# qxiaofan/awesome-orb-slam3-3dvisioncraft-version

Measured on AMD Instinct MI355X. Metric: frames/sec ORB extract+match (752×480, 1000 kp) + LocalBA iters/sec; 1/2/4/8 GPU, higher is better.
Workload: dtype u8

## Files before the change

### awesome-orb-slam3-3dvisioncraft-version_amd/_abi.py

```python
import ctypes as C

import numpy as np

ORB_OK, ORB_E_EMPTY_IMAGE, ORB_E_CAPACITY, ORB_E_INVALID, ORB_E_HIP, ORB_E_NOMEM, ORB_E_ABORTED = 0, -1, -2, -3, -4, -5, -6

KP_DTYPE = np.dtype([("x", "<f4"), ("y", "<f4"), ("size", "<f4"), ("angle", "<f4"), ("response", "<f4"),
                     ("octave", "<i4"), ("class_id", "<i4")])


class OrbxConfig(C.Structure):
    _fields_ = [("nfeatures", C.c_int32), ("scale_factor", C.c_float), ("nlevels", C.c_int32),
                ("ini_th_fast", C.c_int32), ("min_th_fast", C.c_int32)]


TH_HIGH, TH_LOW, HISTO_LENGTH = 100, 50, 30
GRID_COLS, GRID_ROWS = 64, 48
MODE_LOCAL_MAP, MODE_BEST_ONLY, MODE_INIT = 0, 1, 2
Q_VALID, Q_STEREO, Q_HAS_OBS, Q_RIGHT, Q_TWIN = 1, 2, 4, 8, 16

QUERY_DTYPE = np.dtype([("u", "<f4"), ("v", "<f4"), ("radius", "<f4"), ("u_right", "<f4"), ("angle", "<f4"),
                        ("min_level", "<i2"), ("max_level", "<i2"), ("flags", "<u4")])


class GridParams(C.Structure):
# ... 439 lines not shown
    "ORBM_LBA_R_NUM_FIXED_KF": LBA_R_NUM_FIXED_KF, "ORBM_LBA_R_N_POINTS": LBA_R_N_POINTS, "ORBM_LBA_R_N_EDGES": LBA_R_N_EDGES,
    "ORBM_LBA_R_N_MONO": LBA_R_N_MONO, "ORBM_LBA_R_N_STEREO": LBA_R_N_STEREO, "ORBM_LBA_R_N_POSES_REQUIRED": LBA_R_N_POSES_REQUIRED,
    "ORBM_LBA_R_N_POINTS_REQUIRED": LBA_R_N_POINTS_REQUIRED, "ORBM_LBA_R_N_EDGES_REQUIRED": LBA_R_N_EDGES_REQUIRED,
    "ORBM_LBA_R_WORDS": LBA_R_WORDS, "ORBM_LBA_BAD_INDEX": LBA_BAD_INDEX, "ORBM_LBA_UNSUPPORTED": LBA_UNSUPPORTED,
    "ORBM_LBA_OVERFLOW": LBA_OVERFLOW, "ORBM_LBA_EARLY_RETURN": LBA_EARLY_RETURN, "ORBM_LBA_A_FLAGS": LBA_A_FLAGS,
    "ORBM_LBA_A_N_ERASED": LBA_A_N_ERASED, "ORBM_LBA_A_N_WENT_BAD": LBA_A_N_WENT_BAD, "ORBM_LBA_A_N_OBS": LBA_A_N_OBS,
    "ORBM_LBA_A_N_MONO": LBA_A_N_MONO, "ORBM_LBA_A_N_STEREO": LBA_A_N_STEREO, "ORBM_LBA_A_WORDS": LBA_A_WORDS,
    "BOWDB_KF_PRESENT": KF_PRESENT, "BOWDB_COVIS": COVIS, "BOWDB_MAX_CANDIDATES": MAX_CANDIDATES, "BOWDB_L1_NORM": BOWDB_L1_NORM,
    "LBA_EDGE_MONO": EDGE_MONO, "LBA_EDGE_STEREO": EDGE_STEREO, "LBA_EDGE_BODY": EDGE_BODY, "LBA_CAM_PINHOLE": CAM_PINHOLE, "LBA_CAM_KB8": CAM_KB8,
    "LBA_HINT_MONO_PINHOLE": HINT_MONO_PINHOLE, "LBA_HINT_PINHOLE": HINT_PINHOLE, "LIBA_MAX_FREE": LIBA_MAX_FREE, "LIBA_EDGE_CLOSE": EDGE_CLOSE,
}


def _prototypes():
    vp, i32, u32, sz, f32, f64, P = C.c_void_p, C.c_int, C.c_uint, C.c_size_t, C.c_float, C.c_double, C.POINTER
    lba, liba = P(LbaProblem), P(LibaProblem)
    return {
        "orbx_create": (i32, [P(OrbxConfig), i32, i32, i32, i32, P(vp)]),
        "orbx_destroy": (None, [vp]),
        "orbx_last_error": (C.c_char_p, [vp]),
        "orbx_get_tables": (i32, [vp, vp, vp, vp, vp, vp]),
        "orbx_max_keypoints": (i32, [vp]),
        "orbx_extract": (i32, [vp, vp, i32, i32, i32, i32, i32, vp, vp, i32, P(i32), P(i32)]),
        "orbx_extract_view": (i32, [vp, vp, i32, i32, i32, i32, i32, P(vp), P(vp), P(i32), P(i32)]),
        "orbx_set_host_pyramid": (i32, [vp, i32]),
        "orbx_host_pyramid_level": (i32, [vp, i32, P(vp), P(i32), P(i32), P(i32)]),
        "orbx_extract_batch_dev": (i32, [vp, vp, i32, sz, i32, i32, i32, vp, vp, i32, vp, vp]),
        "orbx_pyramid_level": (i32, [vp, i32, i32, P(vp), P(i32), P(i32), P(i32)]),
        "orbx_copy_level": (i32, [vp, i32, i32, i32, vp]),
        "orbx_stereo_matches": (i32, [vp, vp, vp, vp, vp, vp, vp, vp, i32, i32, f32, f32, vp, vp, vp, vp]),
        "orbx_stereo_matches_last": (i32, [vp, vp, f32, f32, vp, vp, i32, P(i32)]),
        "orbx_debug_candidates": (i32, [vp, i32, i32, vp, i32, P(i32)]),
        "orbx_debug_selected": (i32, [vp, i32, i32, vp, i32, P(i32)]),
        "orbx_enable_timing": (i32, [vp, i32]),
        "orbx_last_timing": (i32, [vp, vp]),
        "orbx_last_fast_passes": (i32, [vp, vp, vp, vp]),
        "orbx_last_schedule": (i32, [vp, P(i32), P(i32)]),

        "orbm_hamming": (i32, [vp, i32, vp, i32, i32, vp, vp]),
        "orbm_knn2": (i32, [vp, vp, i32, vp, vp, i32, i32, i32, vp, vp, vp]),
        "orbm_grid_build": (i32, [vp, vp, i32, i32, i32, P(GridParams), vp, vp, vp]),
        "orbm_search_workspace_bytes": (sz, [i32, i32]),
        "orbm_search_by_projection": (i32, [vp, vp, vp, vp, vp, i32, i32, vp, vp, vp, vp, vp, i32, i32, P(SearchParams), vp, vp, vp, vp, vp]),
        "orbm_search_by_bow": (i32, [P(BowSide), vp, P(BowSide), i32, f32, i32, vp, vp, vp]),
        "orbm_search_by_bow_kf": (i32, [P(BowSide), vp, P(BowSide), vp, i32, f32, i32, vp, vp, vp]),
        "orbm_enable_timing": (i32, [i32]),
        "orbm_last_timing": (i32, [vp]),
        "orbm_grid_build_rig": (i32, [vp, vp, vp, i32, i32, i32, P(GridParams), vp, vp, vp]),
        "orbm_search_by_projection_rig": (i32, [vp, vp, vp, vp, vp, i32, i32, vp, vp, vp, vp, vp, i32, i32, P(SearchParams), vp, vp, vp, vp, vp]),
        "orbm_fuse": (i32, [vp, vp, vp, vp, i32, i32, vp, vp, vp, vp, vp, i32, i32, P(FuseParams), vp, vp, vp, vp]),
        "orbm_search_for_triangulation": (i32, [P(TriSide), P(TriSide), vp, i32, i32, i32, i32, vp, vp, vp]),
        "orbm_search_for_triangulation_kb8": (i32, [P(TriSide), P(TriSide), vp, vp, vp, i32, i32, i32, i32, vp, vp, vp]),
        "orbm_mutual_matches": (i32, [vp, vp, vp, vp, i32, i32, i32, vp, vp, vp]),
        "orbm_predict_scale_thresholds": (i32, [f32, i32, vp]),
        "orbm_project_map_points": (i32, [vp, vp, i32, vp, vp, i32, P(ProjectParams), vp, vp, vp, vp, vp, vp, vp, i32, vp]),
        "orbm_refresh_map_points": (i32, [vp, i32, vp, i32, vp, i32, vp, vp, vp, vp, i32, vp, i32, P(RefreshParams), vp, vp, vp]),
        "orbm_create_new_map_points": (i32, [P(NewPtSide), P(NewPtSide), vp, vp, i32, vp, vp, i32, vp, vp, vp, vp, vp, vp]),
        "orbm_append_new_map_points": (i32, [vp, vp, i32, vp, i32, vp, i32, vp, vp, i32, i32, vp, vp, i32, vp, vp, i32, vp, vp]),
        "orbm_local_map_workspace_bytes": (sz, [i32, i32, i32]),
        "orbm_update_local_map": (i32, [P(LocalMapView), vp, P(LocalMapLists), i32, P(LocalMapOut), vp, vp]),
        "orbm_store_local_tracks": (i32, [vp, vp, vp, i32, i32, vp, i32, i32, vp]),
        "orbm_cull_workspace_bytes": (sz, [i32, i32, i32, i32]),
        "orbm_cull_workspace": (i32, [i32, i32, i32, P(CullWorkspaceLayout)]),
        "orbm_cull_keyframes": (i32, [P(LocalMapView), P(CullIn), i32, P(CullOut), vp, vp]),
        "orbm_apply_keyframe_culling": (i32, [P(LocalMapView), P(CullIn), i32, i32, P(CullApply), vp, vp]),
        "orbm_covis_workspace_bytes": (sz, [i32, i32]),
# ... 73 lines not shown
```

### awesome-orb-slam3-3dvisioncraft-version_amd/csrc/orbx_extractor.hip

```cpp
#include <hip/hip_runtime.h>

#include <climits>

#include <cfloat>
#include <cmath>
#include <cstdint>
#include <cstdio>
#include <cstring>
#include <string>
#include <type_traits>
#include <vector>

#include "../../include/orbhip.h"
#include "lds_optin.inc"
#include <mutex>

#define ORBX_MAX_LEVELS 16
#ifdef ORBX_PROF
__device__ unsigned long long g_prof[2][8][256];
#define PROF_DECL unsigned long long prof_t = clock64(), prof_d[8] = {0, 0, 0, 0, 0, 0, 0, 0}
#define PROF_MARK(k, slot) do { const unsigned long long t_ = clock64(); prof_d[slot] += t_ - prof_t; prof_t = t_; } while (0)
#define PROF_FLUSH(k) do { if ((threadIdx.x & 63) < 8) atomicAdd(&g_prof[k][threadIdx.x & 7][(blockIdx.x * 4 + (threadIdx.x >> 6)) & 255], prof_d[threadIdx.x & 7]); } while (0)
#else
#define PROF_DECL do {} while (0)
#define PROF_MARK(k, slot) do {} while (0)
#define PROF_FLUSH(k) do {} while (0)
#endif
#define ORBX_EVENTS_ON(h) ((h)->timing && !(h)->capturing)
#define ORBX_EDGE 19
#define ORBX_MINB 16
#define FAST_QCAP 2048
#define FAST_MAXCELLS 32

static const int8_t h_pattern[1024] = {
#include "orb_pattern.inc"
};
static __constant__ float4 c_patternf[256];
static __constant__ int c_umax[16];
static __constant__ uint32_t c_div16[16] = {0, 65536, 32768, 21846, 16384, 13108, 10923, 9363, 8192, 7282, 6554, 5958, 5462, 5042, 4682, 4370};
static __constant__ uint32_t c_icmask[16][12];

static __device__ __forceinline__ bool xcd_frame_unit_m(const int unitsPerFrame, const uint32_t magic, const int batch, int* frame, int* unit, const int lead = 0, const bool reverse = false) {
    const int xcd = blockIdx.x & 7;
    const uint32_t slot = (uint32_t)(blockIdx.x - lead) >> 3;
    const uint32_t q0 = magic ? (uint32_t)(((unsigned long long)slot * magic) >> 32) : slot / (uint32_t)unitsPerFrame;
    const uint32_t q = reverse ? (uint32_t)((batch + 7) >> 3) - 1u - q0 : q0;
    const int fr = (int)q * 8 + xcd;
    *frame = fr;
    *unit = (int)(slot - q0 * (uint32_t)unitsPerFrame);
    return fr < batch;
}
static inline uint32_t xcd_units_magic(int unitsPerFrame, int batch) {
    const unsigned long long u = (unsigned long long)std::max(unitsPerFrame, 1), slots = u * (unsigned long long)((batch + 7) / 8);
    if (u < 2 || slots * u >= 0x100000000ull) return 0u;
    return (uint32_t)(0x100000000ull / u + 1ull);
}

#include "resize_window.inc"

struct ResizeParams {
    const uint8_t* src; size_t sFrame; int sStride, sw, sh;
    uint8_t* dst; size_t dFrame; int dStride, dw, dh;
    double scale_x, scale_y;
    const int* coef;
    int stripsX, stripsY;
    int stripRows, batch;
    int unitsPerFrame;
    uint32_t unitsMagic;
    int reverse;
    const Resize2Strip* strips;
    const Resize2Row* rows;
    int* ordCand; int* ordOut; uint32_t* ordHostMax; uint32_t* ordRetry; int ordLevels; uint32_t ordTiles;
// ... 646 lines not shown
        } else {
#pragma unroll
            for (int k = 0; k < NS; k++) {
                rr[k] = r; cc[k] = c;
                if (tid + 256 * k < ng) fetch(r, c, w[k]);
                r += dr; c += dc;
                if (c >= gq) { c -= gq; r++; }
            }
        }
#pragma unroll
        for (int k = 0; k < NS; k++)
            if (tid + 256 * k < ng) put(rr[k], cc[k], w[k]);
        for (int i = tid + 256 * NS; i < ng; i += 256) {
            uint32_t wx[5];
            fetch(r, c, wx);
            put(r, c, wx);
            r += dr; c += dc;
            if (c >= gq) { c -= gq; r++; }
        }
        if (tid < 8 + FAST_MAXCELLS) sh[tid] = 0;
        if (tid < detW) {
            const int cell = (int)(mul24((uint32_t)tid, (uint32_t)L.wCellMagic) >> 16);
            const int cellx0 = (int)mul24((uint32_t)cell, (uint32_t)L.wCell);
            const int cx = tid - cellx0, cw = min(L.wCell, detW - cellx0);
            colTab[tid] = (uint8_t)(cell | (cx == 0 ? 0x40 : 0) | (cx + 1 >= cw ? 0x80 : 0));
        }
    }
    PROF_MARK(0, 0);
    __syncthreads();
    PROF_MARK(0, 1);

    const int t0 = PASS == 0 ? P.iniTh : min(P.iniTh, P.minTh);
    const int wave = tid >> 6;
    const int dcol = lane & 31, rsub = lane >> 5;
    uint16_t* q1w = q1 + wave * FAST_Q1W;
    uint16_t* q2w = q2 + wave * (FAST_Q2CAP / 4);
    uint8_t* sbuf = (uint8_t*)q1w;
    static_assert(FAST_Q2CAP / 4 <= 2 * FAST_Q1W, "a wave's scores are parked in its q1 slice");
    static_assert((FAST_Q2CAP / 4 + 1) / 2 + 256 <= FAST_Q1W && FAST_FITS_MAX <= FAST_Q1W, "a row group (<= 256 survivors) queues behind the parked scores");
    static_assert(4 * FAST_PITCH <= 4 * FAST_Q1W * 2, "the fallback's four-row score ring lives in the q1 region");
    static_assert(FAST_CROWS <= 2 && FAST_MAXCELLS / FAST_CROWS <= 16, "a tile's cells are bit 16 * cell row + cell of a 32-bit mask (retry list)");
    int n2w = 0;
    bool ovf = false;
    auto classify = [&](const int i, const bool valid) {
        int ent = 0, S = 0;
        if (valid) {
            ent = q1w[i];
            S = fast_S_pk(img + (dy0 + (ent >> 8)) * pitch + dx0 + (ent & 255), pitch);
        }
        const bool corner = valid && S > t0;
        const unsigned long long mc = __ballot(corner);
        const int nc = __popcll(mc);
        if (n2w + nc <= FAST_Q2CAP / 4) {
            if (corner) {
                const int slot = n2w + __popcll(mc & ((1ull << lane) - 1ull));
                q2w[slot] = (uint16_t)ent;
                sbuf[slot] = (uint8_t)(S - 1);
            }
            n2w += nc;
        } else if (mc) ovf = true;
    };
    uint32_t KB, KG;
    fast_pretest_consts(t0, &KB, &KG);
    const int K = (detH + 7) >> 3;
    uint32_t mask = 0;
    uint32_t colMask[FAST_CROWS];
    if (PASS == 1) {
#pragma unroll
        for (int cr = 0; cr < FAST_CROWS; cr++) {
            colMask[cr] = 0;
#pragma unroll
            for (int t = 0; t < 4; t++)
                colMask[cr] |= (emitMask >> (16 * cr + (colTab[min(4 * dcol + t, detW - 1)] & 63)) & 1u) << (8 * t + 7);
        }
    }
    for (int k = 0; k < K; k++) {
        const int ry = 8 * k + 2 * wave + rsub;
        if (ry < detH && 4 * dcol < detW) {
            const uint32_t* cw = (const uint32_t*)(img + ((dy0 - 3 + ry) & 0xFF) * pitch) + dcol;
            uint32_t bits = fast_pretest4(cw, KB, KG);
            if (PASS == 1) bits &= colMask[cellRowOf(ry)];
            const int nvalid = detW - 4 * dcol;
            if (nvalid < 4) bits &= (1u << (8 * nvalid)) - 1u;
            mask |= bits >> (7 - k);
        }
    }
    {
        const int total = __builtin_amdgcn_readlane(wave_scan_incl(__popc(mask)), 63);
        const bool fits = total <= FAST_FITS_MAX;
        for (int kp = 0; kp < (fits ? 1 : K); kp++) {
            uint32_t m = fits ? mask : mask & (0x01010101u << kp);
            const int cnt = __popc(m);
            const int incl = wave_scan_incl(cnt);
            const int n1 = __builtin_amdgcn_readlane(incl, 63);
            const int qb = fits ? 0 : (n2w + 1) >> 1;
            int slot = qb + incl - cnt;
            const int ent0 = ((2 * wave + rsub) << 8) | (4 * dcol);
            while (m) {
                const int j = __ffs((int)m) - 1;
                m &= m - 1;
                q1w[slot++] = (uint16_t)(ent0 + ((j & 7) << 11) + (j >> 3));
            }
            __builtin_amdgcn_fence(__ATOMIC_RELEASE, "wavefront");
            __builtin_amdgcn_wave_barrier();
            __builtin_amdgcn_fence(__ATOMIC_ACQUIRE, "wavefront");
            for (int i0 = 0; i0 < n1; i0 += 64) classify(qb + i0 + lane, i0 + lane < n1);
            __builtin_amdgcn_fence(__ATOMIC_RELEASE, "wavefront");
            __builtin_amdgcn_wave_barrier();
            __builtin_amdgcn_fence(__ATOMIC_ACQUIRE, "wavefront");
        }
    }
    PROF_MARK(0, 2);
    if (ovf) sh[4] = 1;
    __builtin_amdgcn_fence(__ATOMIC_RELEASE, "wavefront");
    __builtin_amdgcn_wave_barrier();
    __builtin_amdgcn_fence(__ATOMIC_ACQUIRE, "wavefront");
    PROF_MARK(0, 3);
    __syncthreads();
    PROF_MARK(0, 4);
    const bool overflow = sh[4] != 0;
    int* cellCnt = sh + 8;
    auto retry_later = [&](const uint32_t cells) {
        const uint32_t i = atomicAdd(P.retry, 1u);
        P.retry[2 + 2 * i] = (uint32_t)tileIdx | ((uint32_t)frame << 16);
        P.retry[3 + 2 * i] = cells;
    };
    if (overflow && PASS == 0) { if (tid == 0) retry_later(0xFFFFFFFFu); PROF_FLUSH(0); return; }
    if (!overflow) {
        for (int i = tid; i < (P.imgBytes >> 4); i += 256) ((uint4*)smap)[i] = make_uint4(0u, 0u, 0u, 0u);
        __syncthreads();
        for (int i = lane; i < n2w; i += 64) {
            const int slot = i;
            const int ent = q2w[slot];
            const int ry = ent >> 8;
// ... 1111 lines not shown
        int run = 0, v = 0;
        for (int k = 0; k < 32; k++) { if (ctl[1] >= run && ctl[1] < run + sub[k]) v = k; run += sub[k]; }
        ctl[2] = (bin << 5) | v;
    }
    __syncthreads();
    const float median = (float)ctl[2];
    const float thDist = 1.5f * 1.4f * median;
    for (int i = tid; i < N; i += 256) {
        const int s = sad[i];
        if (s >= 0 && !((float)s < thDist)) { P.uRight[(size_t)frame * P.cap + i] = -1.0f; P.depth[(size_t)frame * P.cap + i] = -1.0f; }
    }
}

struct LevelHost {
    int w, h, stride; size_t planeOff, planeBytes;
    int maxBX, maxBY, nCols, nRows, wCell, hCell, nIni; float hX;
    int candCap; size_t candOff; int selCap, selOff;
};

struct orbx_extractor {
    orbx_config cfg; int W, H, maxBatch, device;
    std::vector<float> scale, invScale, sigma2, invSigma2; std::vector<int> nfeat; int umax[16];
    LevelHost lv[ORBX_MAX_LEVELS];
    size_t pyrFrame = 0, candFrame = 0; int selFrame = 0, nodeCap = 0, maxKp = 0;
    int nTiles = 0, nTiles1 = 0, fastImgBytes = 0, octKeyOff = 0, octMerge = 0; size_t fastSmem = 0, octSmem = 0;
    hipStream_t stream = nullptr;
    int32_t* d_rowStart = nullptr; int32_t* d_rowIdx = nullptr; int rowCapAlloc = 0;
    int4* d_chain = nullptr; int chainTiles = 0, chainBuf = 0; size_t chainSmem = 0;
    int* d_coef = nullptr; size_t coefOff[ORBX_MAX_LEVELS] = {0};
    size_t r2StripOff[ORBX_MAX_LEVELS] = {0}, r2RowOff[ORBX_MAX_LEVELS] = {0};
    uint8_t* d_pyr = nullptr; uint32_t* d_cand = nullptr; int* d_candCount = nullptr; uint16_t* d_keyNode = nullptr;
    uint32_t *d_sel = nullptr, *d_selAux = nullptr; int *d_selCount = nullptr, *d_lapCount = nullptr;
    FastTile* d_tiles = nullptr; uint32_t* d_retry = nullptr; int* d_order = nullptr;
    uint32_t* h_retry = nullptr;
    uint32_t fastCalls = 0; int fastLastTwoPass = 0, lastOrdered = 0, lastHeavy = 0;
    uint8_t* d_img = nullptr; int imgStride = 0; orb_keypoint* d_kps1 = nullptr; uint8_t* d_desc1 = nullptr; int32_t* d_counts1 = nullptr;
    uint8_t* d_out1 = nullptr; uint8_t* h_img = nullptr; uint8_t* h_out = nullptr; size_t out1Bytes = 0, kps1Off = 0, desc1Off = 0;
    const uint8_t* lastImages = nullptr; size_t lastFrameStride = 0; int lastRowStride = 0, lastBatch = 0;
    hipEvent_t ev[5] = {nullptr, nullptr, nullptr, nullptr, nullptr}; bool timed = false, timing = false;
    hipGraphExec_t graphExec = nullptr; int graphLap0 = 0, graphLap1 = 0; int graphState = 0;
    bool capturing = false;
    int hostPyr = 0, graphHostPyr = 0; bool hostCall = false, hostPyrValid = false;
    uint8_t* d_bpyr = nullptr; uint8_t* h_bpyr = nullptr; size_t bpyrBytes = 0, bOff[ORBX_MAX_LEVELS] = {0};
    int bPitch[ORBX_MAX_LEVELS] = {0}, bRowStart[ORBX_MAX_LEVELS + 1] = {0};
    hipStream_t stream2 = nullptr; hipEvent_t evFork = nullptr, evJoin = nullptr;
    hipStream_t lastStream = nullptr;
    bool lastSingle = false;
    float* d_stereo1 = nullptr; float* h_stereo1 = nullptr;
    std::string err;
};

static thread_local std::string g_create_err;

static inline int cvRoundF(float v) { return (int)lrintf(v); }
static inline int cvRoundD(double v) { return (int)lrint(v); }

#define HIPCHK(h, call)                                                                                  \
    do {                                                                                                 \
        hipError_t e_ = (call);                                                                          \
        if (e_ != hipSuccess) {                                                                          \
            (h)->err = std::string(#call) + ": " + hipGetErrorString(e_);                                \
            return ORB_E_HIP;                                                                            \
        }                                                                                                \
    } while (0)

static int orbx_fail(orbx_extractor* h, int code, const std::string& msg) {
// ... 48 lines not shown
    std::vector<FastTile> tiles, tiles1;
    size_t pyrOff = 0, candOff = 0; int selOff = 0, maxRows = 0, maxPitch = 0, nodeCap = 0, maxKp = 0;
    for (int l = 0; l < nl; l++) {
        LevelHost& L = h->lv[l];
        L.w = cvRoundF((float)width * h->invScale[l]);
        L.h = cvRoundF((float)height * h->invScale[l]);
        L.stride = (L.w + 63) & ~63;
        L.planeBytes = (size_t)L.stride * L.h;
        L.planeOff = pyrOff;
        if (l > 0) pyrOff += (L.planeBytes + 255) & ~(size_t)255;
        L.maxBX = L.w - ORBX_MINB; L.maxBY = L.h - ORBX_MINB;
        const float fw = (float)(L.maxBX - ORBX_MINB), fh = (float)(L.maxBY - ORBX_MINB);
        L.nCols = (int)(fw / 30.f); L.nRows = (int)(fh / 30.f);
        if (L.nCols < 1 || L.nRows < 1) { orbx_free(h); return orbx_fail(nullptr, ORB_E_INVALID, "image too small for the requested number of pyramid levels"); }
        L.wCell = (int)std::ceil(fw / L.nCols); L.hCell = (int)std::ceil(fh / L.nRows);
        L.nIni = (int)std::round(fw / (L.maxBY - ORBX_MINB));
        if (L.nIni < 1 || L.nCols > 4000) { orbx_free(h); return orbx_fail(nullptr, ORB_E_INVALID, "unsupported aspect ratio (octree needs width/height >= 0.5)"); }
        L.hX = fw / L.nIni;
        int cap = 0;
        const int detWtot = L.w - 2 * ORBX_EDGE, detHtot = L.h - 2 * ORBX_EDGE;
        for (int i = 0; i < L.nRows; i++) {
            const int hh = std::min(L.hCell, detHtot - i * L.hCell);
            if (hh <= 0) continue;
            for (int j = 0; j < L.nCols; j++) {
                const int ww = std::min(L.wCell, detWtot - j * L.wCell);
                if (ww > 0) cap += ((ww + 1) / 2) * ((hh + 1) / 2);
            }
        }
        L.candCap = std::max(cap, 1); L.candOff = candOff; candOff += (size_t)((L.candCap + 3) & ~3);
        L.selCap = std::max(h->nfeat[l], 4 * L.nIni) + 4; L.selOff = selOff; selOff += L.selCap;
        nodeCap = std::max(nodeCap, L.selCap); maxKp += L.selCap;
        if (L.selCap > 60000) { orbx_free(h); return orbx_fail(nullptr, ORB_E_INVALID, "nfeatures per level too large"); }
        const int cpt = std::max(1, std::min(FAST_MAXCELLS / FAST_CROWS, FAST_TW / L.wCell));
        const int nT = (L.nCols + cpt - 1) / cpt, per = (L.nCols + nT - 1) / nT;
        int validRows = 0;
        for (int i = 0; i < L.nRows; i++) if (ORBX_MINB + i * L.hCell < L.maxBY - 3) validRows = i + 1;
        const int crows = (FAST_CROWS * L.hCell <= 64 && 2 * l < nl) ? FAST_CROWS : 1;
        for (int i = 0; i < validRows; i += crows) {
            const int ncr = std::min(crows, validRows - i);
            for (int c0 = 0; c0 < L.nCols; c0 += per) {
                const int n = std::min(per, L.nCols - c0);
                if (ORBX_MINB + c0 * L.wCell >= L.maxBX - 6) continue;
                tiles.push_back(FastTile{(short)(l | (ncr << 8)), (short)i, (short)c0, (short)n});
                maxPitch = std::max(maxPitch, ((n * L.wCell + 6 + 3) + 15) & ~15);
            }
        }
        for (int i = 0; i < validRows; i++)
            for (int c0 = 0; c0 < L.nCols; c0 += per) {
                if (ORBX_MINB + c0 * L.wCell >= L.maxBX - 6) continue;
                tiles1.push_back(FastTile{(short)(l | (1 << 8)), (short)i, (short)c0, (short)std::min(per, L.nCols - c0)});
            }
        maxRows = std::max(maxRows, crows * L.hCell + 6 + crows);
        if (L.hCell > 64) { orbx_free(h); return orbx_fail(nullptr, ORB_E_INVALID, "FAST cell higher than 64 rows"); }
        if (L.wCell > 127) { orbx_free(h); return orbx_fail(nullptr, ORB_E_INVALID, "FAST cell wider than 127 columns"); }
    }
    h->pyrFrame = pyrOff; h->candFrame = candOff; h->selFrame = selOff; h->nodeCap = nodeCap; h->maxKp = maxKp;
    h->nTiles = (int)tiles.size(); h->nTiles1 = (int)tiles1.size();
    if (maxPitch > FAST_PITCH) { orbx_free(h); return orbx_fail(nullptr, ORB_E_INVALID, "FAST tile wider than FAST_PITCH"); }
    h->fastImgBytes = (maxRows * FAST_PITCH + 15) & ~15;
    h->fastSmem = (size_t)h->fastImgBytes + 4 * FAST_Q1W * 2 + FAST_Q2CAP * 2 + FAST_TW + (8 + FAST_MAXCELLS) * 4;
    h->octMerge = (size_t)(256 + 16) * 4 + (size_t)nodeCap * 100 + 16 + 15 <= 150 * 1024 ? 1 : 0;
    h->octKeyOff = (int)(((size_t)(256 + 16) * 4 + (size_t)nodeCap * (h->octMerge ? 100 : 84) + 16 + 15) & ~(size_t)15);
    h->octSmem = (size_t)h->octKeyOff + (size_t)OCT_KEYCAP * 6;
    if (h->octSmem > 150 * 1024) h->octSmem = (size_t)h->octKeyOff;
    if (h->fastSmem > 64 * 1024 || h->octSmem > 150 * 1024) { orbx_free(h); return orbx_fail(nullptr, ORB_E_INVALID, "configuration exceeds the LDS budget"); }

    if (hipSetDevice(device) != hipSuccess) { orbx_free(h); return orbx_fail(nullptr, ORB_E_HIP, "hipSetDevice failed"); }
    if (orb_lds_optin((const void*)k_octree<OCT_T_BATCH>, h->octSmem) != ORB_OK || orb_lds_optin((const void*)k_octree<OCT_T_SINGLE>, h->octSmem) != ORB_OK) {
        orbx_free(h); return orbx_fail(nullptr, ORB_E_HIP, "hipFuncSetAttribute(k_octree) failed");
    }
#define CK(call) do { hipError_t e_ = (call); if (e_ != hipSuccess) { std::string m = std::string(#call) + ": " + hipGetErrorString(e_); orbx_free(h); return orbx_fail(nullptr, e_ == hipErrorOutOfMemory ? ORB_E_NOMEM : ORB_E_HIP, m); } } while (0)
    CK(hipStreamCreateWithFlags(&h->stream, hipStreamNonBlocking));
    for (auto& e : h->ev) CK(hipEventCreate(&e));
    const size_t B = (size_t)max_batch;
    CK(hipMalloc((void**)&h->d_pyr, std::max<size_t>(B * h->pyrFrame, 256)));
    {
        std::vector<int> tab;
        for (int l = 1; l < nl; l++) {
            const int sw = h->lv[l - 1].w, sh = h->lv[l - 1].h, dw = h->lv[l].w, dh = h->lv[l].h;
            const double sx = 1. / ((double)dw / sw), sy = 1. / ((double)dh / sh);
            h->coefOff[l] = tab.size();
            tab.resize(tab.size() + 2 * (size_t)dw + 2 * (size_t)dh);
            int* xs = tab.data() + h->coefOff[l]; int* xw = xs + dw; int* ys = xw + dw; int* yw = ys + dh;
// ... 37 lines not shown
                            x0 = std::min(x0, fx0); x1 = std::max(x1, fx1); y0 = std::min(y0, fy0); y1 = std::max(y1, fy1);
                        }
                        R[l] = make_int4(x0, y0, x1 - x0, y1 - y0);
                        maxArea = std::max(maxArea, (x1 - x0) * (y1 - y0));
                        if (l >= 1) ncoef += 2 * ((x1 - x0) + (y1 - y0));
                        cx0 = x0; cx1 = x1; cy0 = y0; cy1 = y1;
                    }
                    maxCoef = std::max(maxCoef, ncoef);
                }
            h->chainBuf = (maxArea + 15) & ~15;
            h->chainSmem = (size_t)2 * h->chainBuf + (size_t)maxCoef * 4;
            if (h->chainSmem <= 64 * 1024) {
                h->chainTiles = TX * TY;
                CK(hipMalloc((void**)&h->d_chain, reg.size() * sizeof(int4)));
                CK(hipMemcpy(h->d_chain, reg.data(), reg.size() * sizeof(int4), hipMemcpyHostToDevice));
            }
        }
    }
    CK(hipMalloc((void**)&h->d_cand, B * h->candFrame * 4));
    CK(hipMalloc((void**)&h->d_keyNode, B * h->candFrame * 2));
    CK(hipMalloc((void**)&h->d_candCount, B * nl * 4));
    CK(hipMemset(h->d_candCount, 0, B * nl * 4));
    CK(hipMalloc((void**)&h->d_order, B * 4));
    CK(hipMalloc((void**)&h->d_retry, ((size_t)B * tiles.size() * 2 + 2) * 4));
    CK(hipMalloc((void**)&h->d_sel, B * h->selFrame * 4));
    CK(hipMalloc((void**)&h->d_selAux, B * h->selFrame * 4));
    CK(hipMalloc((void**)&h->d_selCount, (B * nl + ORBX_MAX_LEVELS) * 4));
    CK(hipMalloc((void**)&h->d_lapCount, (B * nl + ORBX_MAX_LEVELS) * 4));
    CK(hipMemset(h->d_selCount, 0, (B * nl + ORBX_MAX_LEVELS) * 4));
    CK(hipMemset(h->d_lapCount, 0, (B * nl + ORBX_MAX_LEVELS) * 4));
    tiles.insert(tiles.end(), tiles1.begin(), tiles1.end());
    CK(hipMalloc((void**)&h->d_tiles, tiles.size() * sizeof(FastTile)));
    CK(hipMemcpy(h->d_tiles, tiles.data(), tiles.size() * sizeof(FastTile), hipMemcpyHostToDevice));
    h->imgStride = (width + 63) & ~63;
    CK(hipMalloc((void**)&h->d_img, (size_t)h->imgStride * height));
    h->kps1Off = 64;
    h->desc1Off = (h->kps1Off + (size_t)maxKp * sizeof(orb_keypoint) + 63) & ~(size_t)63;
    h->out1Bytes = h->desc1Off + (size_t)maxKp * 32;
    CK(hipMalloc((void**)&h->d_out1, h->out1Bytes));
    h->d_counts1 = (int32_t*)h->d_out1; h->d_kps1 = (orb_keypoint*)(h->d_out1 + h->kps1Off); h->d_desc1 = h->d_out1 + h->desc1Off;
    CK(hipHostMalloc((void**)&h->h_img, (size_t)h->imgStride * height, hipHostMallocDefault));
    CK(hipHostMalloc((void**)&h->h_retry, 16, hipHostMallocDefault));
    h->h_retry[0] = 0; h->h_retry[1] = 1; h->h_retry[2] = 0; h->h_retry[3] = 0;
    CK(hipHostMalloc((void**)&h->h_out, h->out1Bytes, hipHostMallocDefault));
    {
        static std::mutex constMu;
        static bool constDone[64] = {false};
        std::lock_guard<std::mutex> lock(constMu);
        if (device < 0 || device >= 64 || !constDone[device]) {
            CK(hipMemcpyToSymbol(HIP_SYMBOL(c_umax), h->umax, sizeof(h->umax)));
            float pf[1024];
            for (int i = 0; i < 256; i++) {
                pf[4 * i] = (float)h_pattern[4 * i]; pf[4 * i + 1] = (float)h_pattern[4 * i + 2];
                pf[4 * i + 2] = (float)h_pattern[4 * i + 1]; pf[4 * i + 3] = (float)h_pattern[4 * i + 3];
            }
            CK(hipMemcpyToSymbol(HIP_SYMBOL(c_patternf), pf, sizeof(pf)));
            uint32_t icmask[16][12];
            for (int v = 0; v < 16; v++)
                for (int k = 0; k < 12; k++) {
                    uint32_t m = 0;
                    for (int t = 0; t < 4; t++) { const int u = 4 * k + t - 21; if (u >= -h->umax[v] && u <= h->umax[v]) m |= 0xFFu << (8 * t); }
                    icmask[v][k] = m;
                }
            CK(hipMemcpyToSymbol(HIP_SYMBOL(c_icmask), icmask, sizeof(icmask)));
            if (device >= 0 && device < 64) constDone[device] = true;
        }
// ... 417 lines not shown

extern "C" int orbx_debug_candidates(orbx_handle h, int frame, int level, int32_t* xys, int cap, int* n_out) {
    if (!h || level < 0 || level >= h->cfg.nlevels || frame < 0 || frame >= h->lastBatch || !n_out) return ORB_E_INVALID;
    HIPCHK(h, hipSetDevice(h->device));
    HIPCHK(h, hipStreamSynchronize(h->lastStream));
    int n = 0;
    HIPCHK(h, hipMemcpy(&n, h->d_candCount + (size_t)frame * h->cfg.nlevels + level, 4, hipMemcpyDeviceToHost));
    *n_out = n;
    const int m = std::min(std::min(n, cap), h->lv[level].candCap);
    if (m > 0 && xys) {
        std::vector<uint32_t> tmp(m);
        HIPCHK(h, hipMemcpy(tmp.data(), h->d_cand + (size_t)frame * h->candFrame + h->lv[level].candOff, (size_t)m * 4, hipMemcpyDeviceToHost));
        for (int i = 0; i < m; i++) { xys[3 * i] = tmp[i] & 0xFFF; xys[3 * i + 1] = (tmp[i] >> 12) & 0xFFF; xys[3 * i + 2] = tmp[i] >> 24; }
    }
    return ORB_OK;
}

extern "C" int orbx_debug_selected(orbx_handle h, int frame, int level, int32_t* xys, int cap, int* n_out) {
    if (!h || level < 0 || level >= h->cfg.nlevels || frame < 0 || frame >= h->lastBatch || !n_out) return ORB_E_INVALID;
    HIPCHK(h, hipSetDevice(h->device));
    HIPCHK(h, hipStreamSynchronize(h->lastStream));
    int n = 0;
    HIPCHK(h, hipMemcpy(&n, h->d_selCount + (size_t)frame * h->cfg.nlevels + level, 4, hipMemcpyDeviceToHost));
    *n_out = n;
    const int m = std::min(n, cap);
    if (m > 0 && xys) {
        std::vector<uint32_t> tmp(m);
        HIPCHK(h, hipMemcpy(tmp.data(), h->d_sel + (size_t)frame * h->selFrame + h->lv[level].selOff, (size_t)m * 4, hipMemcpyDeviceToHost));
        for (int i = 0; i < m; i++) { xys[3 * i] = tmp[i] & 0xFFF; xys[3 * i + 1] = (tmp[i] >> 12) & 0xFFF; xys[3 * i + 2] = tmp[i] >> 24; }
    }
    return ORB_OK;
}

#ifdef ORBX_PROF
extern "C" int orbx_debug_prof(unsigned long long* out32, int clear) {
    static unsigned long long z[2 * 8 * 256], r[2 * 8 * 256];
    if (hipDeviceSynchronize() != hipSuccess) return ORB_E_HIP;
    if (hipMemcpyFromSymbol(r, HIP_SYMBOL(g_prof), sizeof(r)) != hipSuccess) return ORB_E_HIP;
    for (int k = 0; k < 16; k++) { out32[k] = 0; for (int i = 0; i < 256; i++) out32[k] += r[k * 256 + i]; }
    if (clear && hipMemcpyToSymbol(HIP_SYMBOL(g_prof), z, sizeof(z)) != hipSuccess) return ORB_E_HIP;
    return ORB_OK;
}
#endif

extern "C" int orbx_last_fast_passes(orbx_handle h, int* two_pass, uint32_t* listed, uint32_t* tiles) {
    if (!h) return ORB_E_INVALID;
    const volatile uint32_t* hr = h->h_retry;
    if (two_pass) *two_pass = h->fastLastTwoPass;
    if (listed) *listed = hr[0];
    if (tiles) *tiles = hr[1];
    return ORB_OK;
}

extern "C" int orbx_last_schedule(orbx_handle h, int* frames_ordered, int* heavy_octree_pass) {
    if (!h) return ORB_E_INVALID;
    if (frames_ordered) *frames_ordered = h->lastOrdered;
    if (heavy_octree_pass) *heavy_octree_pass = h->lastHeavy;
    return ORB_OK;
}

extern "C" int orbx_enable_timing(orbx_handle h, int on) {
    if (!h) return ORB_E_INVALID;
    h->timing = on != 0;
    if (!on) h->timed = false;
    return ORB_OK;
}
// ... 9 lines not shown
```

### include/orbhip.h

```cpp
#ifndef ORBHIP_H
#define ORBHIP_H
#include <stddef.h>
#include <stdint.h>

#ifdef __cplusplus
extern "C" {
#endif

#define ORB_OK 0
#define ORB_E_EMPTY_IMAGE (-1)
#define ORB_E_CAPACITY (-2)
#define ORB_E_INVALID (-3)
#define ORB_E_HIP (-4)
#define ORB_E_NOMEM (-5)
#define ORB_E_ABORTED (-6)

typedef struct orb_keypoint {
    float x, y, size, angle, response;
    int32_t octave, class_id;
} orb_keypoint;

typedef struct orbx_config {
    int32_t nfeatures;
    float scale_factor;
// ... 7 lines not shown
int orbx_create(const orbx_config* cfg, int width, int height, int max_batch, int device, orbx_handle* out);
void orbx_destroy(orbx_handle h);
const char* orbx_last_error(orbx_handle h);

int orbx_get_tables(orbx_handle h, float* scale, float* inv_scale, float* sigma2, float* inv_sigma2,
                    int32_t* features_per_level);
int orbx_max_keypoints(orbx_handle h);

int orbx_extract(orbx_handle h, const uint8_t* image, int width, int height, int stride, int lap0, int lap1,
                 orb_keypoint* kps, uint8_t* desc, int cap, int* n_out, int* mono_index);

int orbx_extract_view(orbx_handle h, const uint8_t* image, int width, int height, int stride, int lap0, int lap1,
                      const orb_keypoint** kps, const uint8_t** desc, int* n_out, int* mono_index);

int orbx_set_host_pyramid(orbx_handle h, int keep);
int orbx_host_pyramid_level(orbx_handle h, int level, const uint8_t** ptr, int* w, int* hgt, int* stride);

int orbx_extract_batch_dev(orbx_handle h, const uint8_t* d_images, int batch, size_t frame_stride, int row_stride,
                           int lap0, int lap1, orb_keypoint* d_kps, uint8_t* d_desc, int cap_per_frame,
                           int32_t* d_counts, void* stream);

int orbx_pyramid_level(orbx_handle h, int frame, int level, const uint8_t** d_ptr, int* w, int* hgt, int* stride);
int orbx_copy_level(orbx_handle h, int frame, int level, int border, uint8_t* out);

int orbx_stereo_matches(orbx_handle left, orbx_handle right, const orb_keypoint* d_kps_l, const uint8_t* d_desc_l,
                        const int32_t* d_counts_l, const orb_keypoint* d_kps_r, const uint8_t* d_desc_r, const int32_t* d_counts_r,
                        int cap_per_frame, int batch, float mb, float mbf, float* d_u_right, float* d_depth, int32_t* d_work,
                        void* stream);

int orbx_stereo_matches_last(orbx_handle left, orbx_handle right, float mb, float mbf, float* u_right, float* depth, int cap, int* n_left);

int orbx_debug_candidates(orbx_handle h, int frame, int level, int32_t* xys, int cap, int* n_out);
int orbx_debug_selected(orbx_handle h, int frame, int level, int32_t* xys, int cap, int* n_out);

int orbx_enable_timing(orbx_handle h, int on);
int orbx_last_timing(orbx_handle h, float* ms5);

int orbx_last_fast_passes(orbx_handle h, int* two_pass, uint32_t* listed, uint32_t* tiles);

int orbx_last_schedule(orbx_handle h, int* frames_ordered, int* heavy_octree_pass);

#define ORBM_TH_HIGH 100
#define ORBM_TH_LOW 50
#define ORBM_HISTO_LENGTH 30
#define ORBM_GRID_COLS 64
#define ORBM_GRID_ROWS 48

int orbm_hamming(const uint8_t* d_q, int nq, const uint8_t* d_t, int nt, int batch, uint16_t* d_out, void* stream);

int orbm_knn2(const uint8_t* d_q, const int32_t* d_nq, int cap_q, const uint8_t* d_t, const int32_t* d_nt, int cap_t,
              int count_stride, int batch, int32_t* d_out_idx, int32_t* d_out_dist, void* stream);

typedef struct orbm_grid_params {
    float min_x, min_y, grid_w_inv, grid_h_inv;
} orbm_grid_params;

int orbm_grid_build(const orb_keypoint* d_kps, const int32_t* d_nkp, int count_stride, int cap_k, int batch,
                    const orbm_grid_params* gp, int32_t* d_grid_start, int32_t* d_grid_idx, void* stream);

typedef struct orbf_camera {
    float fx, fy, cx, cy;
    float dist[5];
} orbf_camera;

int orbf_undistort_keypoints(const orb_keypoint* d_kps, const int32_t* d_nkp, int count_stride, int cap_k, int batch,
                             const orbf_camera* cam, orb_keypoint* d_kps_un, void* stream);
// ... 1067 lines not shown
```

Baseline: 365,300.

## Pack FAST pre-test work into dense tile slots and balance tile widths

The FAST pre-test loop now enumerates 4-pixel slots linearly across the tile, using magic-number division to recover row and column, instead of a fixed 8-row by 32-dword lane mapping. This removes idle lanes on narrow tiles and cuts iterations when rows are shorter than 128 pixels. The per-cell column mask is now fetched with a cross-lane shuffle, and candidate entries are re-encoded from the linear slot. Tile partitioning spreads leftover cells evenly across tiles rather than leaving a short last tile, and a debug API for dumping tiles is added. The change relies on the magic-division table being exact for the range used, and adds shuffle and multiply overhead to each iteration.

```diff
diff --git a/awesome-orb-slam3-3dvisioncraft-version_amd/_abi.py b/awesome-orb-slam3-3dvisioncraft-version_amd/_abi.py
--- a/awesome-orb-slam3-3dvisioncraft-version_amd/_abi.py
+++ b/awesome-orb-slam3-3dvisioncraft-version_amd/_abi.py
@@ -495,6 +495,7 @@
         "orbx_stereo_matches_last": (i32, [vp, vp, f32, f32, vp, vp, i32, P(i32)]),
         "orbx_debug_candidates": (i32, [vp, i32, i32, vp, i32, P(i32)]),
         "orbx_debug_selected": (i32, [vp, i32, i32, vp, i32, P(i32)]),
+        "orbx_debug_fast_tiles": (i32, [vp, i32, vp, i32, P(i32)]),
         "orbx_enable_timing": (i32, [vp, i32]),
         "orbx_last_timing": (i32, [vp, vp]),
         "orbx_last_fast_passes": (i32, [vp, vp, vp, vp]),
diff --git a/awesome-orb-slam3-3dvisioncraft-version_amd/csrc/orbx_extractor.hip b/awesome-orb-slam3-3dvisioncraft-version_amd/csrc/orbx_extractor.hip
--- a/awesome-orb-slam3-3dvisioncraft-version_amd/csrc/orbx_extractor.hip
+++ b/awesome-orb-slam3-3dvisioncraft-version_amd/csrc/orbx_extractor.hip
@@ -37,7 +37,8 @@
 };
 static __constant__ float4 c_patternf[256];
 static __constant__ int c_umax[16];
-static __constant__ uint32_t c_div16[16] = {0, 65536, 32768, 21846, 16384, 13108, 10923, 9363, 8192, 7282, 6554, 5958, 5462, 5042, 4682, 4370};
+static __constant__ uint32_t c_div16[33] = {0, 65536, 32768, 21846, 16384, 13108, 10923, 9363, 8192, 7282, 6554, 5958, 5462, 5042, 4682, 4370, 4096,
+                                            3856, 3641, 3450, 3277, 3121, 2979, 2850, 2731, 2622, 2521, 2428, 2341, 2260, 2185, 2115, 2048};
 static __constant__ uint32_t c_icmask[16][12];
 
 static __device__ __forceinline__ bool xcd_frame_unit_m(const int unitsPerFrame, const uint32_t magic, const int batch, int* frame, int* unit, const int lead = 0, const bool reverse = false) {
@@ -750,7 +751,8 @@
 
     const int t0 = PASS == 0 ? P.iniTh : min(P.iniTh, P.minTh);
     const int wave = tid >> 6;
-    const int dcol = lane & 31, rsub = lane >> 5;
+    const int dwPerRow = (detW + 3) >> 2, nslot = (int)mul24((uint32_t)detH, (uint32_t)dwPerRow);
+    const uint32_t dwm = c_div16[dwPerRow];
     uint16_t* q1w = q1 + wave * FAST_Q1W;
     uint16_t* q2w = q2 + wave * (FAST_Q2CAP / 4);
     uint8_t* sbuf = (uint8_t*)q1w;
@@ -763,10 +765,12 @@
     auto classify = [&](const int i, const bool valid) {
         int ent = 0, S = 0;
         if (valid) {
-            ent = q1w[i];
+            const uint32_t e1 = q1w[i];
+            const uint32_t ry = mul24(e1 & ~3u, dwm) >> 18;
+            ent = (int)((ry << 8) | (e1 - mul24(ry, 4u * (uint32_t)dwPerRow)));
             S = fast_S_pk(img + (dy0 + (ent >> 8)) * pitch + dx0 + (ent & 255), pitch);
         }
-        const bool corner = valid && S > t0;
+        const bool corner = valid && S > t0 && (PASS == 1 || (ent & 255) < detW);
         const unsigned long long mc = __ballot(corner);
         const int nc = __popcll(mc);
         if (n2w + nc <= FAST_Q2CAP / 4) {
@@ -780,27 +784,31 @@
     };
     uint32_t KB, KG;
     fast_pretest_consts(t0, &KB, &KG);
-    const int K = (detH + 7) >> 3;
+    const int K = (nslot + 255) >> 8;
     uint32_t mask = 0;
-    uint32_t colMask[FAST_CROWS];
+    uint32_t colMask = 0;
     if (PASS == 1) {
-#pragma unroll
-        for (int cr = 0; cr < FAST_CROWS; cr++) {
-            colMask[cr] = 0;
-#pragma unroll
-            for (int t = 0; t < 4; t++)
-                colMask[cr] |= (emitMask >> (16 * cr + (colTab[min(4 * dcol + t, detW - 1)] & 63)) & 1u) << (8 * t + 7);
-        }
-    }
-    for (int k = 0; k < K; k++) {
-        const int ry = 8 * k + 2 * wave + rsub;
-        if (ry < detH && 4 * dcol < detW) {
-            const uint32_t* cw = (const uint32_t*)(img + ((dy0 - 3 + ry) & 0xFF) * pitch) + dcol;
+        const int cr = lane >> 5, dc = lane & 31;
+#pragma unroll
+        for (int t = 0; t < 4; t++)
+            if (4 * dc + t < detW) colMask |= (emitMask >> (16 * cr + (colTab[4 * dc + t] & 63)) & 1u) << (8 * t + 7);
+    }
+    const uint32_t rowGap = (uint32_t)pitch - 4u * (uint32_t)dwPerRow;
+    for (int it = 0; it < K; it++) {
+        const uint32_t g4 = 1024u * (uint32_t)it + 4u * (uint32_t)tid;
+#if defined(__HIP_DEVICE_COMPILE__) && !defined(HIP_EMULATED)
+        __builtin_assume(g4 < 8192u);
+#endif
+        const uint32_t ry = mul24(g4, dwm) >> 18;
+        uint32_t cm = 0;
+        if (PASS == 1)
+            cm = (uint32_t)__shfl((int)colMask, (int)(((uint32_t)cellRowOf((int)ry) << 5) | ((g4 - mul24(ry, 4u * (uint32_t)dwPerRow)) >> 2)));
+        if (g4 < 4u * (uint32_t)nslot) {
+            static_assert(dy0 == 3, "the pre-test's base row is the tile's first staged row");
+            const uint32_t* cw = (const uint32_t*)(img + (g4 + mul24(ry, rowGap)));
             uint32_t bits = fast_pretest4(cw, KB, KG);
-            if (PASS == 1) bits &= colMask[cellRowOf(ry)];
-            const int nvalid = detW - 4 * dcol;
-            if (nvalid < 4) bits &= (1u << (8 * nvalid)) - 1u;
-            mask |= bits >> (7 - k);
+            if (PASS == 1) bits &= cm;
+            mask |= bits >> (7 - it);
         }
     }
     {
@@ -813,11 +821,11 @@
             const int n1 = __builtin_amdgcn_readlane(incl, 63);
             const int qb = fits ? 0 : (n2w + 1) >> 1;
             int slot = qb + incl - cnt;
-            const int ent0 = ((2 * wave + rsub) << 8) | (4 * dcol);
+            const int ent0 = tid << 2;
             while (m) {
                 const int j = __ffs((int)m) - 1;
                 m &= m - 1;
-                q1w[slot++] = (uint16_t)(ent0 + ((j & 7) << 11) + (j >> 3));
+                q1w[slot++] = (uint16_t)(ent0 + ((j & 7) << 10) + (j >> 3));
             }
             __builtin_amdgcn_fence(__ATOMIC_RELEASE, "wavefront");
             __builtin_amdgcn_wave_barrier();
@@ -1995,6 +2003,7 @@
     uint8_t* d_pyr = nullptr; uint32_t* d_cand = nullptr; int* d_candCount = nullptr; uint16_t* d_keyNode = nullptr;
     uint32_t *d_sel = nullptr, *d_selAux = nullptr; int *d_selCount = nullptr, *d_lapCount = nullptr;
     FastTile* d_tiles = nullptr; uint32_t* d_retry = nullptr; int* d_order = nullptr;
+    std::vector<FastTile> tilesHost;
     uint32_t* h_retry = nullptr;
     uint32_t fastCalls = 0; int fastLastTwoPass = 0, lastOrdered = 0, lastHeavy = 0;
     uint8_t* d_img = nullptr; int imgStride = 0; orb_keypoint* d_kps1 = nullptr; uint8_t* d_desc1 = nullptr; int32_t* d_counts1 = nullptr;
@@ -2109,23 +2118,25 @@
         nodeCap = std::max(nodeCap, L.selCap); maxKp += L.selCap;
         if (L.selCap > 60000) { orbx_free(h); return orbx_fail(nullptr, ORB_E_INVALID, "nfeatures per level too large"); }
         const int cpt = std::max(1, std::min(FAST_MAXCELLS / FAST_CROWS, FAST_TW / L.wCell));
-        const int nT = (L.nCols + cpt - 1) / cpt, per = (L.nCols + nT - 1) / nT;
+        const int nT = (L.nCols + cpt - 1) / cpt, per = L.nCols / nT, wider = L.nCols % nT;
+        auto tileCell0 = [&](const int t) { return t * per + std::min(t, wider); };
         int validRows = 0;
         for (int i = 0; i < L.nRows; i++) if (ORBX_MINB + i * L.hCell < L.maxBY - 3) validRows = i + 1;
         const int crows = (FAST_CROWS * L.hCell <= 64 && 2 * l < nl) ? FAST_CROWS : 1;
         for (int i = 0; i < validRows; i += crows) {
             const int ncr = std::min(crows, validRows - i);
-            for (int c0 = 0; c0 < L.nCols; c0 += per) {
-                const int n = std::min(per, L.nCols - c0);
+            for (int t = 0; t < nT; t++) {
+                const int c0 = tileCell0(t), n = tileCell0(t + 1) - c0;
                 if (ORBX_MINB + c0 * L.wCell >= L.maxBX - 6) continue;
                 tiles.push_back(FastTile{(short)(l | (ncr << 8)), (short)i, (short)c0, (short)n});
                 maxPitch = std::max(maxPitch, ((n * L.wCell + 6 + 3) + 15) & ~15);
             }
         }
         for (int i = 0; i < validRows; i++)
-            for (int c0 = 0; c0 < L.nCols; c0 += per) {
+            for (int t = 0; t < nT; t++) {
+                const int c0 = tileCell0(t);
                 if (ORBX_MINB + c0 * L.wCell >= L.maxBX - 6) continue;
-                tiles1.push_back(FastTile{(short)(l | (1 << 8)), (short)i, (short)c0, (short)std::min(per, L.nCols - c0)});
+                tiles1.push_back(FastTile{(short)(l | (1 << 8)), (short)i, (short)c0, (short)(tileCell0(t + 1) - c0)});
             }
         maxRows = std::max(maxRows, crows * L.hCell + 6 + crows);
         if (L.hCell > 64) { orbx_free(h); return orbx_fail(nullptr, ORB_E_INVALID, "FAST cell higher than 64 rows"); }
@@ -2229,6 +2240,7 @@
     tiles.insert(tiles.end(), tiles1.begin(), tiles1.end());
     CK(hipMalloc((void**)&h->d_tiles, tiles.size() * sizeof(FastTile)));
     CK(hipMemcpy(h->d_tiles, tiles.data(), tiles.size() * sizeof(FastTile), hipMemcpyHostToDevice));
+    h->tilesHost = tiles;
     h->imgStride = (width + 63) & ~63;
     CK(hipMalloc((void**)&h->d_img, (size_t)h->imgStride * height));
     h->kps1Off = 64;
@@ -2712,6 +2724,20 @@
     return ORB_OK;
 }
 
+extern "C" int orbx_debug_fast_tiles(orbx_handle h, int tall, int32_t* tiles6, int cap, int* n_out) {
+    if (!h || !n_out) return ORB_E_INVALID;
+    const int n = tall ? h->nTiles : h->nTiles1;
+    const FastTile* T = h->tilesHost.data() + (tall ? 0 : h->nTiles);
+    *n_out = n;
+    for (int i = 0; i < std::min(n, cap) && tiles6; i++) {
+        const LevelHost& L = h->lv[T[i].level & 0xFF];
+        const int iniX = ORBX_MINB + T[i].cell0 * L.wCell, maxX = std::min(ORBX_MINB + (T[i].cell0 + T[i].nCells) * L.wCell + 6, L.maxBX);
+        const int32_t rec[6] = {T[i].level & 0xFF, T[i].cellRow, T[i].level >> 8, T[i].cell0, T[i].nCells, maxX - iniX - 6};
+        std::copy(rec, rec + 6, tiles6 + 6 * i);
+    }
+    return ORB_OK;
+}
+
 #ifdef ORBX_PROF
 extern "C" int orbx_debug_prof(unsigned long long* out32, int clear) {
     static unsigned long long z[2 * 8 * 256], r[2 * 8 * 256];
diff --git a/include/orbhip.h b/include/orbhip.h
--- a/include/orbhip.h
+++ b/include/orbhip.h
@@ -63,6 +63,7 @@
 
 int orbx_debug_candidates(orbx_handle h, int frame, int level, int32_t* xys, int cap, int* n_out);
 int orbx_debug_selected(orbx_handle h, int frame, int level, int32_t* xys, int cap, int* n_out);
+int orbx_debug_fast_tiles(orbx_handle h, int tall, int32_t* tiles6, int cap, int* n_out);
 
 int orbx_enable_timing(orbx_handle h, int on);
 int orbx_last_timing(orbx_handle h, float* ms5);
```

After: 365,700 (median of 6 runs). No clear change (+0.1%).
